# nibox/Pose-Estimation-with-Message-Passing-Networks

Measured on AMD Instinct MI355X. Metric: images/sec (640px, HRNet-w48) + MPN edge-updates/sec at 1/2/4/8 MI355X, higher is better.
Workload: dtype f16x3; 1 GPU; c3: 8x17x640x640 heatmaps/GPU -> fully graph -> MPN TypeAware-attn T=3; images_per_gpu=8, global_batch=8, persons_per_image=9, nodes_per_gpu=1224, edges_per_gpu=186048, parallelism=image-sharded x1, batches_in_flight=2, detection_and_node_math=fp32

## Files before the change

### pose-estimation-with-message-passing-networks_amd/csrc/mpn.hip

```cpp
#include <limits.h>

#include <algorithm>
#include <atomic>
#include <type_traits>
#include <map>
#include <mutex>
#include <string>
#include <vector>
#include <string.h>
#include <math.h>

#include "pemp_common.h"

namespace pemp {
namespace {

constexpr int D = 64;
constexpr int LDW = 72;
constexpr int MAXT = 17;
constexpr int EDGE_WAVES = 16;
constexpr int EMB_WAVES = 16, EMB_PER_CU = 1;
constexpr int EMB_MIN_WAVES_EU = EMB_WAVES * EMB_PER_CU / 4 > 1 ? EMB_WAVES * EMB_PER_CU / 4 : 1;
constexpr int RESERVE_CUS_DEFAULT = 64;
constexpr int64_t RESERVE_MIN_EDGES = 65536;
// ... 477 lines not shown
      : "=&v"(hi), "=&v"(lo)
      : "v"(x0), "v"(x1), "v"(s));
}

__device__ __forceinline__ float frag_absmax(const float (&x)[4][4]) {
  float m = 0.0f;
#pragma unroll
  for (int b = 0; b < 4; ++b) m = fmaxf(m, fmaxf(fmaxf(fabsf(x[b][0]), fabsf(x[b][1])), fmaxf(fabsf(x[b][2]), fabsf(x[b][3]))));
  return m;
}

__device__ __forceinline__ bool f16_big(const float (&x)[4][4], float s) {
  return __any(!(frag_absmax(x) * s < F16_BIG));
}

__device__ __forceinline__ float f16_item_scale(float m, float s) {
  m = xmax_rows(m);
  m *= s;
  if (m < F16_BIG) return 1.0f;
  if (!(m <= 3.4028235e38f)) return F16_DOWN;
  int e;
  frexpf(m, &e);
  return ldexpf(1.0f, 14 - e);
}

__device__ __forceinline__ float frag_max_nonneg(const float (&x)[4][4]) {
  int m = 0;
#pragma unroll
  for (int b = 0; b < 4; ++b)
    m = max(m, max(max(__float_as_int(x[b][0]), __float_as_int(x[b][1])), max(__float_as_int(x[b][2]), __float_as_int(x[b][3]))));
  return __int_as_float(m);
}

template <bool NONNEG = false>
__device__ __forceinline__ bool split_f16(const float (&x)[4][4], float s, f16x8_t (&hi)[2], f16x8_t (&lo)[2],
                                          float& sc, float extra = 1.0f) {
  const float m = NONNEG ? frag_max_nonneg(x) : frag_absmax(x);
  const bool big = __any(!(m * s < F16_BIG));
  sc = big ? f16_item_scale(m, s) : 1.0f;
  const float ss = s * sc * extra;
#pragma unroll
  for (int kb = 0; kb < 2; ++kb) {
    uint32_t h[4], l[4];
#pragma unroll
    for (int d = 0; d < 4; ++d)
      split_pair(x[2 * kb + (d >> 1)][2 * (d & 1)], x[2 * kb + (d >> 1)][2 * (d & 1) + 1], ss, h[d], l[d]);
    const u32x4_t hv = {h[0], h[1], h[2], h[3]}, lv = {l[0], l[1], l[2], l[3]};
    hi[kb] = __builtin_bit_cast(f16x8_t, hv);
    lo[kb] = __builtin_bit_cast(f16x8_t, lv);
  }
  return big;
}

template <int OB, bool BIG>
__device__ __forceinline__ void gemm_h3_body(const _Float16* W, const f16x8_t (&hi)[2],
                                             const f16x8_t (&lo)[2], float sc, float (&acc)[OB][4]) {
  const int lane = __lane_id(), i = lane & 15, g = lane >> 4;
  const float isc = BIG ? 1.0f / sc : 1.0f;
#pragma unroll
  for (int ob = 0; ob < OB; ++ob) {
    f32x4 c = {acc[ob][0], acc[ob][1], acc[ob][2], acc[ob][3]};
    if (BIG) c *= sc;
#pragma unroll
    for (int kb = 0; kb < 2; ++kb) {
      const int o = (16 * ob + i) * 2 * LDW + 32 * kb + 8 * g;
      const f16x8_t ah = *reinterpret_cast<const f16x8_t*>(W + o);
      const f16x8_t al = *reinterpret_cast<const f16x8_t*>(W + o + 64);
      c = __builtin_amdgcn_mfma_f32_16x16x32_f16(al, hi[kb], c, 0, 0, 0);
      c = __builtin_amdgcn_mfma_f32_16x16x32_f16(ah, lo[kb], c, 0, 0, 0);
      c = __builtin_amdgcn_mfma_f32_16x16x32_f16(ah, hi[kb], c, 0, 0, 0);
    }
    if (BIG) c *= isc;
    acc[ob][0] = c[0]; acc[ob][1] = c[1]; acc[ob][2] = c[2]; acc[ob][3] = c[3];
  }
}

template <int OB>
__device__ __forceinline__ void gemm_h3(const _Float16* W, const f16x8_t (&hi)[2], const f16x8_t (&lo)[2],
                                        bool big, float sc, float (&acc)[OB][4]) {
  if (__builtin_expect(big, 0)) gemm_h3_body<OB, true>(W, hi, lo, sc, acc);
  else gemm_h3_body<OB, false>(W, hi, lo, 1.0f, acc);
}

template <int PREC>
struct Frag {
  bf16x8_t bh[2], bl[2];
  f16x8_t hh[2], hl[2];
  bool big;
  float sc;
};

template <int PREC, bool NONNEG = false>
__device__ __forceinline__ void prep(const float (&x)[4][4], Frag<PREC>& f) {
  if constexpr (PREC == 1) split_bf16(x, f.bh, f.bl);
  else if constexpr (PREC == 2) f.big = split_f16<NONNEG>(x, dom_inv<PREC>(), f.hh, f.hl, f.sc);
}

template <bool NONNEG = false>
__device__ __forceinline__ void prep_f16_scaled(const float (&x)[4][4], Frag<2>& f, float extra) {
  f.big = split_f16<NONNEG>(x, dom_inv<2>(), f.hh, f.hl, f.sc, extra);
}

template <int PREC>
__device__ __forceinline__ void prep_true(const float (&x)[4][4], Frag<PREC>& f) {
  if constexpr (PREC == 1) split_bf16(x, f.bh, f.bl);
  else if constexpr (PREC == 2) f.big = split_f16(x, 1.0f, f.hh, f.hl, f.sc);
}

template <int PREC, int OB>
__device__ __forceinline__ void gemm_f(const void* W, const float (&x)[4][4], const Frag<PREC>& f, float (&acc)[OB][4]) {
  if constexpr (PREC == 0) gemm_frag<4, OB>(static_cast<const float*>(W), LDW, x, acc);
  else if constexpr (PREC == 1) gemm_bf3<OB>(static_cast<const __bf16*>(W), f.bh, f.bl, acc);
  else gemm_h3<OB>(static_cast<const _Float16*>(W), f.hh, f.hl, f.big, f.sc, acc);
}

__device__ __forceinline__ int interleaved_slot(int row, int rows_per_part, int ld, int part_len) {
  const int part = row >= rows_per_part, r = row - part * rows_per_part;
  return r * ld + part * part_len;
}

__host__ __device__ constexpr int lds_stride(int in_pad) { return (in_pad - 8 + 63) / 64 * 64 + 8; }

struct EmbedLayout {
  int n, prec, w_off[5], stride[5], kb[5], ob[5], b_off[5], relu[5], g_off[5], total;
};

__host__ __device__ constexpr int lds_stride_bf(int in_pad) { return 2 * in_pad + 16; }

__host__ __device__ constexpr EmbedLayout embed_layout_dims(int n, const int* in_dim, const int* out_dim, const int* relu,
                                                            int prec) {
  EmbedLayout L{};
  L.n = n;
  L.prec = prec;
  int off = 0, goff = 0;
  for (int l = 0; l <= L.n; ++l) {
    const int in = l < L.n ? in_dim[l] : 64, out = l < L.n ? out_dim[l] : 64;
    L.ob[l] = (out + 15) / 16;
    L.relu[l] = l < L.n ? relu[l] : 0;
    L.w_off[l] = off;
    if (prec != PEMP_PREC_FP32) {
      L.kb[l] = (in + 31) / 32;
      L.stride[l] = lds_stride_bf(32 * L.kb[l]);
      off += 16 * L.ob[l] * L.stride[l] / 2;
      L.g_off[l] = goff;
      goff += 2 * 16 * L.ob[l] * 32 * L.kb[l];
    } else {
      L.kb[l] = (in + 15) / 16;
      L.stride[l] = lds_stride(16 * L.kb[l]);
      off += 16 * L.ob[l] * L.stride[l];
    }
  }
  for (int l = 0; l <= L.n; ++l) {
    L.b_off[l] = off;
    off += 16 * L.ob[l];
  }
  L.total = off;
  return L;
}

static EmbedLayout embed_layout(const pemp_mlp& m, int prec) {
  int in[4] = {}, out[4] = {}, relu[4] = {};
  const int n = m.n_layers < 4 ? m.n_layers : 4;
  for (int l = 0; l < n; ++l) {
    in[l] = m.layer[l].in_dim;
    out[l] = m.layer[l].out_dim;
    relu[l] = m.layer[l].relu;
// ... 205 lines not shown
          c = __builtin_amdgcn_mfma_f32_16x16x32_bf16(ah, hb[kb], c, 0, 0, 0);
        } else {
          const f16x8_t ah = *reinterpret_cast<const f16x8_t*>(W + o);
          const f16x8_t al = *reinterpret_cast<const f16x8_t*>(W + o + lo_off);
          c = __builtin_amdgcn_mfma_f32_16x16x32_f16(al, hh[kb], c, 0, 0, 0);
          c = __builtin_amdgcn_mfma_f32_16x16x32_f16(ah, lh[kb], c, 0, 0, 0);
          c = __builtin_amdgcn_mfma_f32_16x16x32_f16(ah, hh[kb], c, 0, 0, 0);
        }
      }
#pragma unroll
      for (int r = 0; r < 4; ++r) {
        const float v = c[r] * s_out;
        out[ob][r] = relu ? fmaxf(v, 0.0f) : v;
      }
    } else {
#pragma unroll
      for (int r = 0; r < 4; ++r) out[ob][r] = 0.0f;
    }
  }
}

template <int KB, bool NONNEG>
__device__ __forceinline__ bool split_f16_kb(const float (&x)[4][4], float s, f16x8_t (&hi)[2], f16x8_t (&lo)[2],
                                             float& sc) {
  float m;
  if constexpr (NONNEG) {
    int mi = 0;
#pragma unroll
    for (int b = 0; b < 2 * KB; ++b)
      mi = max(mi, max(max(__float_as_int(x[b][0]), __float_as_int(x[b][1])), max(__float_as_int(x[b][2]), __float_as_int(x[b][3]))));
    m = __int_as_float(mi);
  } else {
    m = 0.0f;
#pragma unroll
    for (int b = 0; b < 2 * KB; ++b)
      m = fmaxf(m, fmaxf(fmaxf(fabsf(x[b][0]), fabsf(x[b][1])), fmaxf(fabsf(x[b][2]), fabsf(x[b][3]))));
  }
  const bool big = __any(!(m * s < F16_BIG));
  sc = big ? f16_item_scale(m, s) : 1.0f;
  const float ss = s * sc;
#pragma unroll
  for (int kb = 0; kb < KB; ++kb) {
    uint32_t h[4], l[4];
#pragma unroll
    for (int d = 0; d < 4; ++d)
      split_pair(x[2 * kb + (d >> 1)][2 * (d & 1)], x[2 * kb + (d >> 1)][2 * (d & 1) + 1], ss, h[d], l[d]);
    const u32x4_t hv = {h[0], h[1], h[2], h[3]}, lv = {l[0], l[1], l[2], l[3]};
    hi[kb] = __builtin_bit_cast(f16x8_t, hv);
    lo[kb] = __builtin_bit_cast(f16x8_t, lv);
  }
  return big;
}

template <int KB32, int OB, bool RELU, bool NONNEG, bool BIG>
__device__ __forceinline__ void layer_h3_body(const _Float16* W, int ldw, const float* bias, const f16x8_t (&hh)[2],
                                              const f16x8_t (&lh)[2], float sc, float (&out)[4][4]) {
  const int lane = __lane_id(), i = lane & 15, g = lane >> 4;
  constexpr int lo_off = 32 * KB32;
  const float isc = BIG ? 1.0f / sc : 1.0f;
#pragma unroll
  for (int ob = 0; ob < 4; ++ob) {
    if (ob < OB) {
      const float4 bb = ld4(bias + 16 * ob + 4 * g);
      f32x4 c = {bb.x, bb.y, bb.z, bb.w};
      if (BIG) c *= sc;
#pragma unroll
      for (int kb = 0; kb < KB32; ++kb) {
        const int o = (16 * ob + i) * ldw + 32 * kb + 8 * g;
        const f16x8_t ah = *reinterpret_cast<const f16x8_t*>(W + o);
        const f16x8_t al = *reinterpret_cast<const f16x8_t*>(W + o + lo_off);
        c = __builtin_amdgcn_mfma_f32_16x16x32_f16(al, hh[kb], c, 0, 0, 0);
        c = __builtin_amdgcn_mfma_f32_16x16x32_f16(ah, lh[kb], c, 0, 0, 0);
        c = __builtin_amdgcn_mfma_f32_16x16x32_f16(ah, hh[kb], c, 0, 0, 0);
      }
      if (BIG) c *= isc;
#pragma unroll
      for (int r = 0; r < 4; ++r) out[ob][r] = RELU ? fmaxf(c[r], 0.0f) : c[r];
    } else {
#pragma unroll
      for (int r = 0; r < 4; ++r) out[ob][r] = 0.0f;
    }
  }
}

template <int KB32, int OB, bool RELU, bool NONNEG, bool IN_DOM>
__device__ __forceinline__ void layer_h3(const float* smz, const EmbedLayout& Lo, int l, const float (&in)[4][4],
                                         float (&out)[4][4], Frag<2>* split_out = nullptr) {
  const _Float16* W = reinterpret_cast<const _Float16*>(smz + Lo.w_off[l]);
  const float* bias = smz + Lo.b_off[l];
  f16x8_t hh[2], lh[2];
  float sc;
  const bool big = split_f16_kb<KB32, NONNEG>(in, IN_DOM ? dom_inv<2>() : 1.0f, hh, lh, sc);
  if (split_out) {
    split_out->hh[0] = hh[0]; split_out->hh[1] = hh[1];
    split_out->hl[0] = lh[0]; split_out->hl[1] = lh[1];
    split_out->big = big;
    split_out->sc = sc;
  }
  if (__builtin_expect(big, 0)) layer_h3_body<KB32, OB, RELU, NONNEG, true>(W, Lo.stride[l], bias, hh, lh, sc, out);
  else layer_h3_body<KB32, OB, RELU, NONNEG, false>(W, Lo.stride[l], bias, hh, lh, 1.0f, out);
}

template <int PREC, bool COMP = false>
__device__ __forceinline__ void embed_tile_fixed(const float* smz, const EmbedLayout& Lo, float (&x)[4][4],
                                                 float (&y)[4][4], Frag<PREC>& fx) {
  if constexpr (PREC == 2 && COMP) {
    layer_h3<1, 2, true, false, false>(smz, Lo, 0, x, y);
    layer_h3<1, 4, true, true, true>(smz, Lo, 1, y, x);
    layer_h3<2, 4, true, true, true>(smz, Lo, 2, x, y);
    layer_h3<2, 4, false, true, true>(smz, Lo, 3, y, x, &fx);
  } else if constexpr (PREC == 2) {
    layer_h3<1, 2, true, false, false>(smz, Lo, 0, x, y);
    layer_h3<1, 4, true, true, true>(smz, Lo, 1, y, x);
    layer_h3<2, 4, true, true, true>(smz, Lo, 2, x, y);
    layer_h3<2, 4, false, true, true>(smz, Lo, 3, y, x);
    layer_h3<2, 4, false, false, true>(smz, Lo, 4, x, y, &fx);
  } else {
    layer_fixed<PREC, 1, 2>(smz, Lo, 0, x, y);
    layer_fixed<PREC, 1, 4>(smz, Lo, 1, y, x);
    layer_fixed<PREC, 2, 4>(smz, Lo, 2, x, y);
    layer_fixed<PREC, 2, 4>(smz, Lo, 3, y, x);
    layer_fixed<PREC, 2, 4, true>(smz, Lo, 4, x, y, &fx);
  }
}

static bool embed_fixed_shape(const EmbedLayout& L) {
  static const int kb[5] = {1, 1, 2, 2, 2}, ob[5] = {2, 4, 4, 4, 4}, relu[5] = {1, 1, 1, 0, 0};
  if (L.prec == PEMP_PREC_FP32 || L.n != 4) return false;
  for (int l = 0; l < 5; ++l)
    if (L.kb[l] != kb[l] || L.ob[l] != ob[l] || (L.relu[l] != 0) != (relu[l] != 0)) return false;
  return true;
}
static bool embed_composed(const EmbedLayout& L, int prec, const pemp_mpn_weights& w) {
  return prec == PEMP_PREC_F16X3 && embed_fixed_shape(L) && w.emb_comp_bf && w.emb_comp_b;
}

template <int PREC>
__device__ __forceinline__ void stage_tile64(float* dst, const float* w32, int64_t ld32, const uint16_t* wbf) {
  if (PREC == 0) {
    for (int idx = threadIdx.x; idx < D * 16; idx += blockDim.x) {
      const int row = idx >> 4, c4 = (idx & 15) * 4;
      *reinterpret_cast<float4*>(&dst[row * LDW + c4]) = ld4(w32 + row * ld32 + c4);
    }
  } else {
    __bf16* db = reinterpret_cast<__bf16*>(dst);
    for (int idx = threadIdx.x; idx < 2 * D * 8; idx += blockDim.x) {
      const int row = idx >> 3, c8 = (idx & 7) * 8;
      *reinterpret_cast<uint4*>(&db[interleaved_slot(row, D, 2 * LDW, D) + c8]) =
          *reinterpret_cast<const uint4*>(wbf + row * D + c8);
    }
  }
}

template <int PREC, bool FIXED>
__device__ __forceinline__ void embed_stage(float* dst, int tid, int nthreads, const pemp_mlp& emb, const EmbedLayout& Lo,
                                            const uint16_t* __restrict__ emb_bf, const float* __restrict__ q0_w,
                                            const float* __restrict__ q0_b, const float* __restrict__ e1_w,
                                            const uint16_t* __restrict__ e1_bf, const uint16_t* __restrict__ comp_bf,
                                            const float* __restrict__ comp_b) {
  const bool comp = FIXED && PREC == 2 && comp_bf && comp_b;
  float* d64 = dst + Lo.total;
  if (comp) {
  } else if (PREC == 0) {
    for (int idx = tid; idx < D * 16; idx += nthreads) {
      const int row = idx >> 4, c4 = (idx & 15) * 4;
      *reinterpret_cast<float4*>(&d64[row * LDW + c4]) = ld4(e1_w + row * D + c4);
    }
  } else {
    __bf16* db = reinterpret_cast<__bf16*>(d64);
// ... 49 lines not shown
void edge_embed_kernel(pemp_mlp emb, EmbedLayout Lo,
                                                                     const uint16_t* __restrict__ emb_bf,
                                                                     const float* __restrict__ ea, int A,
                                                                     const int* __restrict__ s_orig, int64_t E,
                                                                     const float* __restrict__ q0_w,
                                                                     const float* __restrict__ q0_b,
                                                                     const float* __restrict__ e1_w,
                                                                     const uint16_t* __restrict__ e1_bf,
                                                                     float* __restrict__ r0, float* __restrict__ q0,
                                                                     const int64_t* __restrict__ ne,
                                                                     const float* __restrict__ img,
                                                                     const uint16_t* __restrict__ comp_bf,
                                                                     const float* __restrict__ comp_b) {
  constexpr bool FIXED = FX >= 1, COMP = FX == 2;
  extern __shared__ __attribute__((aligned(16))) float sm[];
  if (ne) E = ne[1];
  const int lane = threadIdx.x & 63, wave = threadIdx.x >> 6, c = lane & 15, g = lane >> 4;
  if (img) {
    dma_to_lds(sm, img, COMP ? embed_comp_floats(Lo) : embed_image_floats(Lo));
    lds_drain();
  } else {
    embed_stage<PREC, FIXED>(sm, threadIdx.x, 64 * EMB_WAVES, emb, Lo, emb_bf, q0_w, q0_b, e1_w, e1_bf,
                             COMP ? comp_bf : nullptr, COMP ? comp_b : nullptr);
  }
  __syncthreads();
  const int64_t gw = (int64_t)blockIdx.x * EMB_WAVES + wave, nw = (int64_t)gridDim.x * EMB_WAVES;
  const int first = __builtin_amdgcn_readfirstlane((int)(E * gw / nw));
  const int end = __builtin_amdgcn_readfirstlane((int)(E * (gw + 1) / nw));
  const rsrc_t rs_ea = make_rsrc(ea, (int)E * A * 4), rs_orig = make_rsrc(s_orig, (int)E * 4);
  const rsrc_t rs_q0 = make_rsrc(q0, (int)E * 256), rs_r0 = make_rsrc(r0, (int)E * 256);
  int o_next = first < end ? bld1(rs_orig, 4 * min(first + c, end - 1)) : 0;
  float ea_n[2][4];
  if (FIXED && first < end) {
    load_edge_attr32(rs_ea, A, o_next, ea_n);
    o_next = bld1(rs_orig, 4 * min(first + 16 + c, end - 1));
  }
  for (int base = first; base < end; base += 16) {
    int z = 0;
    asm volatile("" : "+s"(z));
    const float* smz = sm + z;
    const int p = base + c;
    const bool valid = p < end;
    float x[4][4], y[4][4];
    if constexpr (FIXED) {
      ea_mask(A, ea_n, x);
      load_edge_attr32(rs_ea, A, o_next, ea_n);
      o_next = bld1(rs_orig, 4 * min(base + 32 + c, end - 1));
    } else {
      const int o = o_next;
      o_next = bld1(rs_orig, 4 * min(base + 16 + c, end - 1));
      load_edge_attr(rs_ea, A, o, x);
    }
    Frag<PREC> fx;
    const int vo = valid ? p * 256 + 16 * g : OOB_VOFF;
    if constexpr (COMP) {
      embed_tile_fixed<PREC, true>(smz, Lo, x, y, fx);
#pragma unroll
      for (int ob = 0; ob < 4; ++ob) bst4(rs_q0, vo + 64 * ob, x[ob][0], x[ob][1], x[ob][2], x[ob][3]);
      const float* br = smz + Lo.b_off[4];
#pragma unroll
      for (int ob = 0; ob < 4; ++ob) {
        const float4 bb = ld4(br + 16 * ob + 4 * g);
        x[ob][0] = bb.x; x[ob][1] = bb.y; x[ob][2] = bb.z; x[ob][3] = bb.w;
      }
      gemm_f<PREC, 4>(smz + Lo.w_off[4], y, fx, x);
#pragma unroll
      for (int ob = 0; ob < 4; ++ob) bst4(rs_r0, vo + 64 * ob, x[ob][0], x[ob][1], x[ob][2], x[ob][3]);
      continue;
    }
    if constexpr (FIXED) {
      embed_tile_fixed<PREC>(smz, Lo, x, y, fx);
    } else {
      embed_tile<PREC>(smz, Lo, x, y);
      if (PREC == 2) {
#pragma unroll
        for (int ob = 0; ob < 4; ++ob)
#pragma unroll
          for (int r = 0; r < 4; ++r) y[ob][r] *= dom<PREC>();
      }
      prep_true<PREC>(x, fx);
    }
#pragma unroll
    for (int ob = 0; ob < 4; ++ob) bst4(rs_q0, vo + 64 * ob, y[ob][0], y[ob][1], y[ob][2], y[ob][3]);
    gemm_f<PREC, 4>(smz + Lo.total, x, fx, y);
#pragma unroll
    for (int ob = 0; ob < 4; ++ob) bst4(rs_r0, vo + 64 * ob, y[ob][0], y[ob][1], y[ob][2], y[ob][3]);
  }
}

struct EdgeStepArgs {
  int64_t N, E;
  int T, t_nt_ld;
  const int4* ranges;
  const int *s_src, *s_dst, *s_orig;
  const float *NT, *Q0, *r_cur;
  float* r_next;
  const float* img;
  int64_t img_stride;
  float* agg;
  pemp_mlp head;
  float* edge_logits;
  int write_next;
  unsigned long long* stamps;
  const int64_t* ne;
  int rec;
  const float* ea;
  int A;
  const float* emb_img;
};

#ifdef PEMP_STAMPS
#define EDGE_STAMP(k)                                                                               \
  do {                                                                                              \
    if (a.stamps && lane == 0) {                                                                    \
      unsigned long long t_;                                                                        \
      asm volatile("s_memrealtime %0\n\ts_waitcnt lgkmcnt(0)" : "=s"(t_)::"memory");                \
      a.stamps[16 * ((int64_t)blockIdx.x * NW + wave) + (k)] = t_;                                  \
    }                                                                                               \
  } while (0)
#else
#define EDGE_STAMP(k) \
  do {                \
  } while (0)
#endif
// ... 377 lines not shown
  if (FIRST && first < end) o_next = bld1(rs_orig, 4 * min(first + c, end - 1));
  {
    const float* src = a.img + (int64_t)t * a.img_stride + SKIP;
    constexpr int PIECES = IMG_F / 256, TAIL = IMG_F - PIECES * 256;
    for (int k = wave; k < PIECES; k += NW)
      dma16(src + 256 * k + 4 * lane, img + 256 * k);
    if (TAIL && wave == NW - 1 && 4 * lane < TAIL)
      *reinterpret_cast<float4*>(&img[256 * PIECES + 4 * lane]) = ld4(src + 256 * PIECES + 4 * lane);
    if constexpr (FIRST) {
      constexpr int EP = EMB_F / 256, ET = EMB_F - EP * 256;
      for (int k = wave; k < EP; k += NW) dma16(a.emb_img + 256 * k + 4 * lane, rbuf + 256 * k);
      if (ET && wave == NW - 2 && 4 * lane < ET)
        *reinterpret_cast<float4*>(&rbuf[256 * EP + 4 * lane]) = ld4(a.emb_img + 256 * EP + 4 * lane);
    }
  }
  if (FIRST) {
    if (first < end) {
      load_edge_attr32(rs_ea, a.A, o_next, ea_n);
      o_next = bld1(rs_orig, 4 * min(first + 16 + c, end - 1));
    }
  } else if (first < end) {
    gather_nt(dst_n, src_n, true);
    dma_rows(rs_r, first, mybuf, lane);
    if (HEAD == 1) orig_t = bld1(rs_orig, 4 * min(first + c, end - 1));
  }
  __syncthreads();
  EDGE_STAMP(1);
  EDGE_STAMP(2);
  const int seg_first = (rflags & RANGE_CONT_IN) ? sdst_id(__builtin_amdgcn_readfirstlane(dst_n)) : -1;
  const rsrc_t rs_next = make_rsrc(a.r_next, E * 256);
  const rsrc_t rs_agg = make_rsrc(a.agg, (int)a.N * T * 256);
  const u32x4v_s rw_r = rsrc_words(a.r_cur, end * 256);
  const u32x4v_s rw_q = rsrc_words(a.Q0, end * 256);
  const rsrc_t rs_q0 = make_rsrc(a.Q0, FIRST ? E * 256 : 0);
  const bool store_next = MID && a.write_next;

  float cacc[4][4];
  float cM = 0.f, cl = 0.f;
  bool have_carry = false;
  int tile_no = 0;
  for (int base = first; base < end; base += 16, ++tile_no) {
    if (tile_no < 4) EDGE_STAMP(3 + 3 * tile_no);
    if (tile_no == 0) __builtin_amdgcn_s_setprio(3);
    else if (tile_no == 1) __builtin_amdgcn_s_setprio(2);
    else if (tile_no == 2) __builtin_amdgcn_s_setprio(1);
    else if (tile_no == 3) __builtin_amdgcn_s_setprio(0);
    int z = 0;
    asm volatile("" : "+s"(z));
    const float* W1 = img + z;
    const float* W2 = img + z + D * LDW - SKIP;
    const float* WM = img + z + 2 * D * LDW - SKIP;
    const float* UW = img + z + 3 * D * LDW - SKIP;
    const float* hwz = hw + z;
    const int p = base + c;
    const bool valid = p < end;
    const int dst = dst_n, src = src_n;
    const bool more = base + 16 < end;
    dst_n = dst_nn;
    src_n = src_nn;
    constexpr int NG = 12 + (HEAD == 1 ? 1 : 0);
    if (!FIRST && tile_no > 0) {
      if (store_next) dma_wait<8 + NG>();
      else dma_wait<4 + NG>();
    }
    float h[4][4], m[4][4], q0r[4][4];
    float4 rr[4];
    if constexpr (FIRST) {
      const float* smz = rbuf + z;
      float y[4][4], r0[4][4];
      Frag<PREC> fx;
      ea_mask(a.A, ea_n, q0r, g + z);
      load_edge_attr32(rs_ea, a.A, o_next, ea_n, g + z);
      o_next = bld1(rs_orig, 4 * min(base + 32 + c, end - 1));
      embed_tile_fixed<PREC, true>(smz, ELO, q0r, y, fx);
      const int vq0 = valid ? p * 256 + 16 * g : OOB_VOFF;
#pragma unroll
      for (int ob = 0; ob < 4; ++ob) bst4(rs_q0, vq0 + 64 * ob, q0r[ob][0], q0r[ob][1], q0r[ob][2], q0r[ob][3]);
      gather_ab(dst, src);
      const float* br = smz + ELO.b_off[4];
#pragma unroll
      for (int ob = 0; ob < 4; ++ob) {
        const float4 bb = ld4(br + 16 * ob + 4 * g);
        r0[ob][0] = bb.x; r0[ob][1] = bb.y; r0[ob][2] = bb.z; r0[ob][3] = bb.w;
      }
      gemm_f<PREC, 4>(smz + ELO.w_off[4], y, fx, r0);
#pragma unroll
      for (int ob = 0; ob < 4; ++ob) rr[ob] = make_float4(r0[ob][0], r0[ob][1], r0[ob][2], r0[ob][3]);
    } else {
      const int cz = c + z, rowb = 64 * cz + 4 * g;
#pragma unroll
      for (int ob = 0; ob < 4; ++ob) rr[ob] = ld4(mybuf + (rowb ^ (16 * (ob ^ (cz & 3)))));
    }
    const int vq = p * 256 + 16 * g;
    const int orig = orig_t;
    if (MID && !FIRST) {
#pragma unroll
      for (int ob = 0; ob < 4; ++ob) asm volatile("" ::"v"(xa[ob].x), "v"(xb[ob].x), "v"(xp[ob].x));
      if (store_next) dma_rows_async(rw_q, base, mybuf, lane);
    }
    {
      const int qn = min(base + 32 + c, end - 1);
      dst_nn = bld1(rs_dst, 4 * qn);
      src_nn = bld1(rs_src, 4 * qn);
    }
    float ab[4][4];
#pragma unroll
    for (int ob = 0; ob < 4; ++ob) {
      if (EPT) {
        h[ob][0] = rr[ob].x; h[ob][1] = rr[ob].y; h[ob][2] = rr[ob].z; h[ob][3] = rr[ob].w;
        ab[ob][0] = xa[ob].x + xb[ob].x; ab[ob][1] = xa[ob].y + xb[ob].y;
        ab[ob][2] = xa[ob].z + xb[ob].z; ab[ob][3] = xa[ob].w + xb[ob].w;
      } else {
        h[ob][0] = rr[ob].x + xa[ob].x + xb[ob].x; h[ob][1] = rr[ob].y + xa[ob].y + xb[ob].y;
        h[ob][2] = rr[ob].z + xa[ob].z + xb[ob].z; h[ob][3] = rr[ob].w + xa[ob].w + xb[ob].w;
      }
    }
    if constexpr (FIRST) {
#pragma unroll
      for (int ob = 0; ob < 4; ++ob) asm volatile("" ::"v"(h[ob][0]), "v"(h[ob][1]), "v"(h[ob][2]), "v"(h[ob][3]));
      gather_p(dst);
#pragma unroll
      for (int ob = 0; ob < 4; ++ob) {
        const float4 q = bld4(rs_q0, min(p, end - 1) * 256 + 16 * g + 64 * ob);
        q0r[ob][0] = q.x; q0r[ob][1] = q.y; q0r[ob][2] = q.z; q0r[ob][3] = q.w;
      }
    }
    if (!MID) {
#pragma unroll
      for (int ob = 0; ob < 4; ++ob) asm volatile("" ::"v"(xa[ob].x), "v"(xb[ob].x), "v"(xp[ob].x));
      if (HEAD == 1) asm volatile("" ::"v"(orig));
      if (more) dma_rows_async(rw_r, base + 16, mybuf, lane);
    }
#pragma unroll
    for (int ob = 0; ob < 4; ++ob) {
      m[ob][0] = xp[ob].x; m[ob][1] = xp[ob].y; m[ob][2] = xp[ob].z; m[ob][3] = xp[ob].w;
    }
#ifdef PEMP_STAMPS
    asm volatile("" ::"v"(h[0][0]), "v"(h[3][3]));
    if (tile_no < 4) EDGE_STAMP(4 + 3 * tile_no);
#endif
    relu_frag<4>(h);
    float ep[4][4];
#pragma unroll
    for (int ob = 0; ob < 4; ++ob) {
      const float4 b2 = ld4(vec + 16 * ob + 4 * g);
      ep[ob][0] = b2.x; ep[ob][1] = b2.y; ep[ob][2] = b2.z; ep[ob][3] = b2.w;
      if (EPT) { ep[ob][0] += ab[ob][0]; ep[ob][1] += ab[ob][1]; ep[ob][2] += ab[ob][2]; ep[ob][3] += ab[ob][3]; }
    }
    {
      Frag<PREC> fh;
      prep<PREC, true>(h, fh);
      gemm_f<PREC, 4>(W2, h, fh, ep);
    }
    relu_frag<4>(ep);
    float av = 0.f;
    if (AGG == PEMP_AGGR_ATTN) {
#pragma unroll
      for (int ob = 0; ob < 4; ++ob) {
        const float4 w = ld4(vec + D + 16 * ob + 4 * g);
        av = fmaf(w.x, ep[ob][0], av); av = fmaf(w.y, ep[ob][1], av);
        av = fmaf(w.z, ep[ob][2], av); av = fmaf(w.w, ep[ob][3], av);
      }
      av = xsum_rows(av);
      av += vec[z + 2 * D];
    }
    const int seg = valid ? sdst_id(dst) : -1 - c;
    const Chunks ck = chunks_of(dst, c, min(end - 1 - base, 15), valid);
    const bool carry_in = have_carry;
    float M = 0.f, pe = 1.0f;
    if (AGG == PEMP_AGGR_ATTN) {
#if PEMP_ASM_SCANS
      M = chunk_max_asm(av, chunk_masks(ck));
#else
      M = seg_bcast_tail_max(seg_max(av, ck.d), ck.u);
#endif
      if (carry_in && ck.d == c) M = fmaxf(M, cM);
      pe = pemp_exp(av - M);
    }
    if (HEAD == 2) {
      float h1[4][4], h2[4][4];
#pragma unroll
      for (int ob = 0; ob < 4; ++ob)
#pragma unroll
        for (int r = 0; r < 4; ++r) h1[ob][r] = ep[ob][r] * dom_inv<PREC>();
      mlp_frag<4>(a.head, h1, h2);
      if (valid && g == 0)
        __builtin_amdgcn_raw_buffer_store_b32(__float_as_uint(h1[0][0]), make_rsrc(logits, E * 4),
                                              4 * a.s_orig[p], 0, 0);
    }
    Frag<PREC> fe;
    prep<PREC, true>(ep, fe);
    if (MID && !FIRST) {
      if (store_next) {
        dma_wait<2>();
        const int cz = c + z, rowb = 64 * cz + 4 * g;
#pragma unroll
        for (int ob = 0; ob < 4; ++ob) {
          const float4 q = ld4(mybuf + (rowb ^ (16 * (ob ^ (cz & 3)))));
          q0r[ob][0] = q.x; q0r[ob][1] = q.y; q0r[ob][2] = q.z; q0r[ob][3] = q.w;
        }
      }
      if (more) dma_rows_async(rw_r, base + 16, mybuf, lane);
    }
    if (MID && a.write_next) {
      gemm_f<PREC, 4>(W1, ep, fe, q0r);
      const int vn = valid ? vq : OOB_VOFF;
#pragma unroll
      for (int ob = 0; ob < 4; ++ob) bst4(rs_next, vn + 64 * ob, q0r[ob][0], q0r[ob][1], q0r[ob][2], q0r[ob][3]);
    }
    if (HEAD == 1) {
      const float* hb = hb_l + z;
      float h1[4][4], h2[2][4];
#pragma unroll
      for (int ob = 0; ob < 4; ++ob) {
        const float4 bb = ld4(hb + 16 * ob + 4 * g);
        h1[ob][0] = bb.x; h1[ob][1] = bb.y; h1[ob][2] = bb.z; h1[ob][3] = bb.w;
      }
      gemm_f<PREC, 4>(hwz, ep, fe, h1);
      relu_frag<4>(h1);
#pragma unroll
      for (int ob = 0; ob < 2; ++ob) {
        const float4 bb = ld4(hb + D + 16 * ob + 4 * g);
        h2[ob][0] = bb.x; h2[ob][1] = bb.y; h2[ob][2] = bb.z; h2[ob][3] = bb.w;
      }
      {
        Frag<PREC> f1;
        prep<PREC, true>(h1, f1);
        gemm_f<PREC, 2>(hwz + D * LDW, h1, f1, h2);
      }
      relu_frag<2>(h2);
      float lg = 0.f;
#pragma unroll
      for (int ob = 0; ob < 2; ++ob) {
        const float4 w = ld4(hb + D + 32 + 16 * ob + 4 * g);
        lg = fmaf(w.x, h2[ob][0], lg); lg = fmaf(w.y, h2[ob][1], lg);
        lg = fmaf(w.z, h2[ob][2], lg); lg = fmaf(w.w, h2[ob][3], lg);
      }
      lg = xsum_rows(lg);
      if (valid && g == 0)
        __builtin_amdgcn_raw_buffer_store_b32(__float_as_uint(lg + hb[D + 64]), make_rsrc(logits, E * 4),
                                              4 * orig, 0, 0);
    }
    gemm_f<PREC, 4>(WM, ep, fe, m);
    relu_frag<4>(m);
    if (UPD) {
      float u[4][4];
#pragma unroll
      for (int ob = 0; ob < 4; ++ob)
#pragma unroll
        for (int r = 0; r < 4; ++r) u[ob][r] = 0.0f;
      Frag<PREC> fm;
      if constexpr (PE_FOLD) prep_f16_scaled<true>(m, fm, pe);
      else prep<PREC, true>(m, fm);
      gemm_f<PREC, 4>(UW, m, fm, u);
#pragma unroll
      for (int ob = 0; ob < 4; ++ob)
#pragma unroll
        for (int r = 0; r < 4; ++r) m[ob][r] = u[ob][r];
    }

    float l = (AGG == PEMP_AGGR_ATTN) ? pe : 1.0f;
    float v[4][4];
#pragma unroll
    for (int ob = 0; ob < 4; ++ob)
#pragma unroll
      for (int r = 0; r < 4; ++r) v[ob][r] = (AGG == PEMP_AGGR_ATTN && !PE_FOLD) ? pe * m[ob][r] : m[ob][r];
    if (carry_in && c == 0) {
      if (AGG == PEMP_AGGR_ATTN) {
        const float f = pemp_exp(cM - M);
        l += cl * f;
#pragma unroll
        for (int ob = 0; ob < 4; ++ob)
#pragma unroll
          for (int r = 0; r < 4; ++r) v[ob][r] = fmaf(cacc[ob][r], f, v[ob][r]);
      } else {
        l += cl;
#pragma unroll
        for (int ob = 0; ob < 4; ++ob)
#pragma unroll
          for (int r = 0; r < 4; ++r)
            v[ob][r] = (AGG == PEMP_AGGR_MAX) ? fmaxf(v[ob][r], cacc[ob][r]) : v[ob][r] + cacc[ob][r];
      }
    }
    const ScanMask smk = scan_mask(ck.d);
    {
      if (AGG == PEMP_AGGR_ATTN || AGG == PEMP_AGGR_MEAN) l = seg_sum(l, smk);
#pragma unroll
      for (int ob = 0; ob < 4; ++ob)
#pragma unroll
        for (int r = 0; r < 4; ++r) v[ob][r] = (AGG == PEMP_AGGR_MAX) ? seg_max(v[ob][r], ck.d) : seg_sum(v[ob][r], smk);
    }
    const int seg15 = __builtin_amdgcn_readlane(seg, 15);
    const bool carry_out = more && sdst_id(__builtin_amdgcn_readlane(dst_n, 0)) == seg15;
    if (carry_out) {
      cl = readlane_f(l, 15);
      cM = readlane_f(M, 15);
#pragma unroll
      for (int ob = 0; ob < 4; ++ob)
#pragma unroll
        for (int r = 0; r < 4; ++r) cacc[ob][r] = dppf<DPP_SHL15>(v[ob][r], 0.0f);
    }
    have_carry = carry_out;
    {
      const float inv = ((AGG == PEMP_AGGR_ATTN) ? pemp_rcp(l + 1e-12f) : (AGG == PEMP_AGGR_MEAN) ? pemp_rcp(l) : 1.0f) *
                        dom_inv<PREC>();
      const bool out = valid && ck.tail && !(carry_out && c == 15);
      const bool pin = seg == seg_first;
// ... 2393 lines not shown
```

Baseline: 35510 images/s.

## Software-pipeline LDS weight fragment reads across chained f16x3 MFMA GEMMs

Restructures the f16x3 split-precision GEMM so that weight fragments for the next step are read from LDS while the current MFMAs run. The first fragment of the following layer's weights is also prefetched across GEMM boundaries in both the embedding MLP and the edge update chain. sched_group_barrier hints interleave ds_reads with MFMAs. The big-scale path becomes a runtime multiply instead of a separate template instantiation. This aims to hide LDS latency between dependent MFMA chains, at the cost of higher VGPR pressure from holding prefetched fragments, which could lower occupancy.

```diff
diff --git a/pose-estimation-with-message-passing-networks_amd/csrc/mpn.hip b/pose-estimation-with-message-passing-networks_amd/csrc/mpn.hip
--- a/pose-estimation-with-message-passing-networks_amd/csrc/mpn.hip
+++ b/pose-estimation-with-message-passing-networks_amd/csrc/mpn.hip
@@ -553,34 +553,68 @@
   return big;
 }
 
-template <int OB, bool BIG>
-__device__ __forceinline__ void gemm_h3_body(const _Float16* W, const f16x8_t (&hi)[2],
-                                             const f16x8_t (&lo)[2], float sc, float (&acc)[OB][4]) {
+struct H3Step {
+  f16x8_t ah[2], al[2];
+};
+__device__ __forceinline__ void h3_read(const _Float16* W, int ldw, int lo_off, int q, int kb, H3Step& f) {
   const int lane = __lane_id(), i = lane & 15, g = lane >> 4;
-  const float isc = BIG ? 1.0f / sc : 1.0f;
+  const int o = (32 * q + i) * ldw + 32 * kb + 8 * g;
+#pragma unroll
+  for (int j = 0; j < 2; ++j) f.al[j] = *reinterpret_cast<const f16x8_t*>(W + o + 16 * j * ldw + lo_off);
+#pragma unroll
+  for (int j = 0; j < 2; ++j) f.ah[j] = *reinterpret_cast<const f16x8_t*>(W + o + 16 * j * ldw);
+}
+
+template <int KB, int OB, bool PRE, bool NEXT>
+__device__ __forceinline__ void h3_chain(const _Float16* W, int ldw, int lo_off, const f16x8_t (&hi)[2],
+                                         const f16x8_t (&lo)[2], f32x4 (&c)[OB], H3Step& io,
+                                         const _Float16* Wn, int ldwn, int lo_offn) {
+  static_assert(OB % 2 == 0, "two output blocks per step");
+  constexpr int Q = OB / 2, S = KB * Q;
+  H3Step f[S + 1];
+  if (PRE) f[0] = io;
+  else h3_read(W, ldw, lo_off, 0, 0, f[0]);
+#pragma unroll
+  for (int s = 0; s < S; ++s) {
+    const int kb = s / Q, q = s % Q;
+    if (s + 1 < S) h3_read(W, ldw, lo_off, (s + 1) % Q, (s + 1) / Q, f[s + 1]);
+    else if (NEXT) h3_read(Wn, ldwn, lo_offn, 0, 0, f[s + 1]);
+#pragma unroll
+    for (int j = 0; j < 2; ++j) c[2 * q + j] = __builtin_amdgcn_mfma_f32_16x16x32_f16(f[s].al[j], hi[kb], c[2 * q + j], 0, 0, 0);
+#pragma unroll
+    for (int j = 0; j < 2; ++j) c[2 * q + j] = __builtin_amdgcn_mfma_f32_16x16x32_f16(f[s].ah[j], lo[kb], c[2 * q + j], 0, 0, 0);
+#pragma unroll
+    for (int j = 0; j < 2; ++j) c[2 * q + j] = __builtin_amdgcn_mfma_f32_16x16x32_f16(f[s].ah[j], hi[kb], c[2 * q + j], 0, 0, 0);
+    constexpr int MFMA = 0x008, DS_READ = 0x100;
+    const bool rd = s + 1 < S || NEXT;
+    __builtin_amdgcn_sched_group_barrier(MFMA, 2, 0);
+    if (rd) __builtin_amdgcn_sched_group_barrier(DS_READ, 2, 0);
+    __builtin_amdgcn_sched_group_barrier(MFMA, 4, 0);
+    if (rd) __builtin_amdgcn_sched_group_barrier(DS_READ, 2, 0);
+  }
+  if (NEXT) io = f[S];
+}
+
+template <int OB, bool PRE = false, bool NEXT = false>
+__device__ __forceinline__ void gemm_h3(const _Float16* W, const f16x8_t (&hi)[2], const f16x8_t (&lo)[2],
+                                        bool big, float sc, float (&acc)[OB][4], H3Step& io, const _Float16* Wn) {
+  f32x4 c[OB];
+#pragma unroll
+  for (int ob = 0; ob < OB; ++ob) c[ob] = f32x4{acc[ob][0], acc[ob][1], acc[ob][2], acc[ob][3]};
+  if (__builtin_expect(big, 0)) {
+#pragma unroll
+    for (int ob = 0; ob < OB; ++ob) c[ob] *= sc;
+  }
+  h3_chain<2, OB, PRE, NEXT>(W, 2 * LDW, 64, hi, lo, c, io, Wn, 2 * LDW, 64);
+  if (__builtin_expect(big, 0)) {
+    const float isc = 1.0f / sc;
+#pragma unroll
+    for (int ob = 0; ob < OB; ++ob) c[ob] *= isc;
+  }
 #pragma unroll
   for (int ob = 0; ob < OB; ++ob) {
-    f32x4 c = {acc[ob][0], acc[ob][1], acc[ob][2], acc[ob][3]};
-    if (BIG) c *= sc;
-#pragma unroll
-    for (int kb = 0; kb < 2; ++kb) {
-      const int o = (16 * ob + i) * 2 * LDW + 32 * kb + 8 * g;
-      const f16x8_t ah = *reinterpret_cast<const f16x8_t*>(W + o);
-      const f16x8_t al = *reinterpret_cast<const f16x8_t*>(W + o + 64);
-      c = __builtin_amdgcn_mfma_f32_16x16x32_f16(al, hi[kb], c, 0, 0, 0);
-      c = __builtin_amdgcn_mfma_f32_16x16x32_f16(ah, lo[kb], c, 0, 0, 0);
-      c = __builtin_amdgcn_mfma_f32_16x16x32_f16(ah, hi[kb], c, 0, 0, 0);
-    }
-    if (BIG) c *= isc;
-    acc[ob][0] = c[0]; acc[ob][1] = c[1]; acc[ob][2] = c[2]; acc[ob][3] = c[3];
-  }
-}
-
-template <int OB>
-__device__ __forceinline__ void gemm_h3(const _Float16* W, const f16x8_t (&hi)[2], const f16x8_t (&lo)[2],
-                                        bool big, float sc, float (&acc)[OB][4]) {
-  if (__builtin_expect(big, 0)) gemm_h3_body<OB, true>(W, hi, lo, sc, acc);
-  else gemm_h3_body<OB, false>(W, hi, lo, 1.0f, acc);
+    acc[ob][0] = c[ob][0]; acc[ob][1] = c[ob][1]; acc[ob][2] = c[ob][2]; acc[ob][3] = c[ob][3];
+  }
 }
 
 template <int PREC>
@@ -612,7 +646,28 @@
 __device__ __forceinline__ void gemm_f(const void* W, const float (&x)[4][4], const Frag<PREC>& f, float (&acc)[OB][4]) {
   if constexpr (PREC == 0) gemm_frag<4, OB>(static_cast<const float*>(W), LDW, x, acc);
   else if constexpr (PREC == 1) gemm_bf3<OB>(static_cast<const __bf16*>(W), f.bh, f.bl, acc);
-  else gemm_h3<OB>(static_cast<const _Float16*>(W), f.hh, f.hl, f.big, f.sc, acc);
+  else {
+    H3Step io;
+    gemm_h3<OB>(static_cast<const _Float16*>(W), f.hh, f.hl, f.big, f.sc, acc, io, nullptr);
+  }
+}
+
+template <int PREC, bool AHEAD = true>
+struct WPre {
+  H3Step s;
+};
+template <int PREC, bool AHEAD>
+__device__ __forceinline__ void wpre(const void* W, WPre<PREC, AHEAD>& p) {
+  if constexpr (PREC == 2 && AHEAD) h3_read(static_cast<const _Float16*>(W), 2 * LDW, 64, 0, 0, p.s);
+}
+
+template <int PREC, int OB, bool NEXT, bool AHEAD>
+__device__ __forceinline__ void gemm_fp(const void* W, const float (&x)[4][4], const Frag<PREC>& f, float (&acc)[OB][4],
+                                        WPre<PREC, AHEAD>& p, const void* Wn = nullptr) {
+  if constexpr (PREC == 2 && AHEAD)
+    gemm_h3<OB, true, NEXT>(static_cast<const _Float16*>(W), f.hh, f.hl, f.big, f.sc, acc, p.s,
+                            static_cast<const _Float16*>(Wn));
+  else gemm_f<PREC, OB>(W, x, f, acc);
 }
 
 __device__ __forceinline__ int interleaved_slot(int row, int rows_per_part, int ld, int part_len) {
@@ -924,40 +979,39 @@
   return big;
 }
 
-template <int KB32, int OB, bool RELU, bool NONNEG, bool BIG>
+template <int KB32, int OB, bool RELU, int KBN>
 __device__ __forceinline__ void layer_h3_body(const _Float16* W, int ldw, const float* bias, const f16x8_t (&hh)[2],
-                                              const f16x8_t (&lh)[2], float sc, float (&out)[4][4]) {
-  const int lane = __lane_id(), i = lane & 15, g = lane >> 4;
-  constexpr int lo_off = 32 * KB32;
-  const float isc = BIG ? 1.0f / sc : 1.0f;
-#pragma unroll
-  for (int ob = 0; ob < 4; ++ob) {
-    if (ob < OB) {
-      const float4 bb = ld4(bias + 16 * ob + 4 * g);
-      f32x4 c = {bb.x, bb.y, bb.z, bb.w};
-      if (BIG) c *= sc;
-#pragma unroll
-      for (int kb = 0; kb < KB32; ++kb) {
-        const int o = (16 * ob + i) * ldw + 32 * kb + 8 * g;
-        const f16x8_t ah = *reinterpret_cast<const f16x8_t*>(W + o);
-        const f16x8_t al = *reinterpret_cast<const f16x8_t*>(W + o + lo_off);
-        c = __builtin_amdgcn_mfma_f32_16x16x32_f16(al, hh[kb], c, 0, 0, 0);
-        c = __builtin_amdgcn_mfma_f32_16x16x32_f16(ah, lh[kb], c, 0, 0, 0);
-        c = __builtin_amdgcn_mfma_f32_16x16x32_f16(ah, hh[kb], c, 0, 0, 0);
-      }
-      if (BIG) c *= isc;
-#pragma unroll
-      for (int r = 0; r < 4; ++r) out[ob][r] = RELU ? fmaxf(c[r], 0.0f) : c[r];
-    } else {
-#pragma unroll
-      for (int r = 0; r < 4; ++r) out[ob][r] = 0.0f;
-    }
-  }
-}
-
-template <int KB32, int OB, bool RELU, bool NONNEG, bool IN_DOM>
+                                              const f16x8_t (&lh)[2], bool big, float sc, float (&out)[4][4],
+                                              H3Step& io, const _Float16* Wn, int ldwn) {
+  const int lane = __lane_id(), g = lane >> 4;
+  f32x4 c[OB];
+#pragma unroll
+  for (int ob = 0; ob < OB; ++ob) {
+    const float4 bb = ld4(bias + 16 * ob + 4 * g);
+    c[ob] = f32x4{bb.x, bb.y, bb.z, bb.w};
+  }
+  if (__builtin_expect(big, 0)) {
+#pragma unroll
+    for (int ob = 0; ob < OB; ++ob) c[ob] *= sc;
+  }
+  h3_chain<KB32, OB, true, (KBN > 0)>(W, ldw, 32 * KB32, hh, lh, c, io, Wn, ldwn, 32 * KBN);
+  if (__builtin_expect(big, 0)) {
+    const float isc = 1.0f / sc;
+#pragma unroll
+    for (int ob = 0; ob < OB; ++ob) c[ob] *= isc;
+  }
+#pragma unroll
+  for (int ob = 0; ob < 4; ++ob)
+#pragma unroll
+    for (int r = 0; r < 4; ++r) {
+      const float v = c[ob < OB ? ob : 0][r];
+      out[ob][r] = ob < OB ? (RELU ? fmaxf(v, 0.0f) : v) : 0.0f;
+    }
+}
+
+template <int KB32, int OB, bool RELU, bool NONNEG, bool IN_DOM, int KBN>
 __device__ __forceinline__ void layer_h3(const float* smz, const EmbedLayout& Lo, int l, const float (&in)[4][4],
-                                         float (&out)[4][4], Frag<2>* split_out = nullptr) {
+                                         float (&out)[4][4], H3Step& io, Frag<2>* split_out = nullptr) {
   const _Float16* W = reinterpret_cast<const _Float16*>(smz + Lo.w_off[l]);
   const float* bias = smz + Lo.b_off[l];
   f16x8_t hh[2], lh[2];
@@ -969,24 +1023,28 @@
     split_out->big = big;
     split_out->sc = sc;
   }
-  if (__builtin_expect(big, 0)) layer_h3_body<KB32, OB, RELU, NONNEG, true>(W, Lo.stride[l], bias, hh, lh, sc, out);
-  else layer_h3_body<KB32, OB, RELU, NONNEG, false>(W, Lo.stride[l], bias, hh, lh, 1.0f, out);
+  const int ln = KBN > 0 ? l + 1 : l;
+  layer_h3_body<KB32, OB, RELU, KBN>(W, Lo.stride[l], bias, hh, lh, big, sc, out, io,
+                                     reinterpret_cast<const _Float16*>(smz + Lo.w_off[ln]), Lo.stride[ln]);
 }
 
 template <int PREC, bool COMP = false>
 __device__ __forceinline__ void embed_tile_fixed(const float* smz, const EmbedLayout& Lo, float (&x)[4][4],
-                                                 float (&y)[4][4], Frag<PREC>& fx) {
+                                                 float (&y)[4][4], Frag<PREC>& fx, WPre<PREC>& wp) {
+  if constexpr (PREC == 2) {
+    h3_read(reinterpret_cast<const _Float16*>(smz + Lo.w_off[0]), Lo.stride[0], 32, 0, 0, wp.s);
+  }
   if constexpr (PREC == 2 && COMP) {
-    layer_h3<1, 2, true, false, false>(smz, Lo, 0, x, y);
-    layer_h3<1, 4, true, true, true>(smz, Lo, 1, y, x);
-    layer_h3<2, 4, true, true, true>(smz, Lo, 2, x, y);
-    layer_h3<2, 4, false, true, true>(smz, Lo, 3, y, x, &fx);
+    layer_h3<1, 2, true, false, false, 1>(smz, Lo, 0, x, y, wp.s);
+    layer_h3<1, 4, true, true, true, 2>(smz, Lo, 1, y, x, wp.s);
+    layer_h3<2, 4, true, true, true, 2>(smz, Lo, 2, x, y, wp.s);
+    layer_h3<2, 4, false, true, true, 2>(smz, Lo, 3, y, x, wp.s, &fx);
   } else if constexpr (PREC == 2) {
-    layer_h3<1, 2, true, false, false>(smz, Lo, 0, x, y);
-    layer_h3<1, 4, true, true, true>(smz, Lo, 1, y, x);
-    layer_h3<2, 4, true, true, true>(smz, Lo, 2, x, y);
-    layer_h3<2, 4, false, true, true>(smz, Lo, 3, y, x);
-    layer_h3<2, 4, false, false, true>(smz, Lo, 4, x, y, &fx);
+    layer_h3<1, 2, true, false, false, 1>(smz, Lo, 0, x, y, wp.s);
+    layer_h3<1, 4, true, true, true, 2>(smz, Lo, 1, y, x, wp.s);
+    layer_h3<2, 4, true, true, true, 2>(smz, Lo, 2, x, y, wp.s);
+    layer_h3<2, 4, false, true, true, 2>(smz, Lo, 3, y, x, wp.s);
+    layer_h3<2, 4, false, false, true, 0>(smz, Lo, 4, x, y, wp.s, &fx);
   } else {
     layer_fixed<PREC, 1, 2>(smz, Lo, 0, x, y);
     layer_fixed<PREC, 1, 4>(smz, Lo, 1, y, x);
@@ -1142,9 +1200,10 @@
       load_edge_attr(rs_ea, A, o, x);
     }
     Frag<PREC> fx;
+    WPre<PREC> wp;
     const int vo = valid ? p * 256 + 16 * g : OOB_VOFF;
     if constexpr (COMP) {
-      embed_tile_fixed<PREC, true>(smz, Lo, x, y, fx);
+      embed_tile_fixed<PREC, true>(smz, Lo, x, y, fx, wp);
 #pragma unroll
       for (int ob = 0; ob < 4; ++ob) bst4(rs_q0, vo + 64 * ob, x[ob][0], x[ob][1], x[ob][2], x[ob][3]);
       const float* br = smz + Lo.b_off[4];
@@ -1153,13 +1212,13 @@
         const float4 bb = ld4(br + 16 * ob + 4 * g);
         x[ob][0] = bb.x; x[ob][1] = bb.y; x[ob][2] = bb.z; x[ob][3] = bb.w;
       }
-      gemm_f<PREC, 4>(smz + Lo.w_off[4], y, fx, x);
+      gemm_fp<PREC, 4, false>(smz + Lo.w_off[4], y, fx, x, wp);
 #pragma unroll
       for (int ob = 0; ob < 4; ++ob) bst4(rs_r0, vo + 64 * ob, x[ob][0], x[ob][1], x[ob][2], x[ob][3]);
       continue;
     }
     if constexpr (FIXED) {
-      embed_tile_fixed<PREC>(smz, Lo, x, y, fx);
+      embed_tile_fixed<PREC>(smz, Lo, x, y, fx, wp);
     } else {
       embed_tile<PREC>(smz, Lo, x, y);
       if (PREC == 2) {
@@ -1643,6 +1702,7 @@
     const float* WM = img + z + 2 * D * LDW - SKIP;
     const float* UW = img + z + 3 * D * LDW - SKIP;
     const float* hwz = hw + z;
+    const float* WA = HEAD == 1 ? hwz : WM;
     const int p = base + c;
     const bool valid = p < end;
     const int dst = dst_n, src = src_n;
@@ -1656,6 +1716,7 @@
     }
     float h[4][4], m[4][4], q0r[4][4];
     float4 rr[4];
+    WPre<PREC, !EPT && HEAD != 2> wp;
     if constexpr (FIRST) {
       const float* smz = rbuf + z;
       float y[4][4], r0[4][4];
@@ -1663,7 +1724,7 @@
       ea_mask(a.A, ea_n, q0r, g + z);
       load_edge_attr32(rs_ea, a.A, o_next, ea_n, g + z);
       o_next = bld1(rs_orig, 4 * min(base + 32 + c, end - 1));
-      embed_tile_fixed<PREC, true>(smz, ELO, q0r, y, fx);
+      embed_tile_fixed<PREC, true>(smz, ELO, q0r, y, fx, wp);
       const int vq0 = valid ? p * 256 + 16 * g : OOB_VOFF;
 #pragma unroll
       for (int ob = 0; ob < 4; ++ob) bst4(rs_q0, vq0 + 64 * ob, q0r[ob][0], q0r[ob][1], q0r[ob][2], q0r[ob][3]);
@@ -1674,7 +1735,7 @@
         const float4 bb = ld4(br + 16 * ob + 4 * g);
         r0[ob][0] = bb.x; r0[ob][1] = bb.y; r0[ob][2] = bb.z; r0[ob][3] = bb.w;
       }
-      gemm_f<PREC, 4>(smz + ELO.w_off[4], y, fx, r0);
+      gemm_fp<PREC, 4, true>(smz + ELO.w_off[4], y, fx, r0, wp, W2);
 #pragma unroll
       for (int ob = 0; ob < 4; ++ob) rr[ob] = make_float4(r0[ob][0], r0[ob][1], r0[ob][2], r0[ob][3]);
     } else {
@@ -1730,6 +1791,7 @@
     asm volatile("" ::"v"(h[0][0]), "v"(h[3][3]));
     if (tile_no < 4) EDGE_STAMP(4 + 3 * tile_no);
 #endif
+    if (!FIRST) wpre(W2, wp);
     relu_frag<4>(h);
     float ep[4][4];
 #pragma unroll
@@ -1741,7 +1803,7 @@
     {
       Frag<PREC> fh;
       prep<PREC, true>(h, fh);
-      gemm_f<PREC, 4>(W2, h, fh, ep);
+      gemm_fp<PREC, 4, true>(W2, h, fh, ep, wp, MID ? W1 : WA);
     }
     relu_frag<4>(ep);
     float av = 0.f;
@@ -1793,11 +1855,15 @@
       }
       if (more) dma_rows_async(rw_r, base + 16, mybuf, lane);
     }
+    constexpr bool W1_NEXT = FIRST || HEAD == 1;
     if (MID && a.write_next) {
-      gemm_f<PREC, 4>(W1, ep, fe, q0r);
+      gemm_fp<PREC, 4, W1_NEXT>(W1, ep, fe, q0r, wp, WA);
       const int vn = valid ? vq : OOB_VOFF;
 #pragma unroll
       for (int ob = 0; ob < 4; ++ob) bst4(rs_next, vn + 64 * ob, q0r[ob][0], q0r[ob][1], q0r[ob][2], q0r[ob][3]);
+      if (!W1_NEXT) wpre(WA, wp);
+    } else if (MID) {
+      wpre(WA, wp);
     }
     if (HEAD == 1) {
       const float* hb = hb_l + z;
@@ -1807,7 +1873,7 @@
         const float4 bb = ld4(hb + 16 * ob + 4 * g);
         h1[ob][0] = bb.x; h1[ob][1] = bb.y; h1[ob][2] = bb.z; h1[ob][3] = bb.w;
       }
-      gemm_f<PREC, 4>(hwz, ep, fe, h1);
+      gemm_fp<PREC, 4, true>(hwz, ep, fe, h1, wp, hwz + D * LDW);
       relu_frag<4>(h1);
 #pragma unroll
       for (int ob = 0; ob < 2; ++ob) {
@@ -1817,7 +1883,7 @@
       {
         Frag<PREC> f1;
         prep<PREC, true>(h1, f1);
-        gemm_f<PREC, 2>(hwz + D * LDW, h1, f1, h2);
+        gemm_fp<PREC, 2, true>(hwz + D * LDW, h1, f1, h2, wp, WM);
       }
       relu_frag<2>(h2);
       float lg = 0.f;
@@ -1832,7 +1898,7 @@
         __builtin_amdgcn_raw_buffer_store_b32(__float_as_uint(lg + hb[D + 64]), make_rsrc(logits, E * 4),
                                               4 * orig, 0, 0);
     }
-    gemm_f<PREC, 4>(WM, ep, fe, m);
+    gemm_fp<PREC, 4, (UPD != 0)>(WM, ep, fe, m, wp, UW);
     relu_frag<4>(m);
     if (UPD) {
       float u[4][4];
@@ -1843,7 +1909,7 @@
       Frag<PREC> fm;
       if constexpr (PE_FOLD) prep_f16_scaled<true>(m, fm, pe);
       else prep<PREC, true>(m, fm);
-      gemm_f<PREC, 4>(UW, m, fm, u);
+      gemm_fp<PREC, 4, false>(UW, m, fm, u, wp);
 #pragma unroll
       for (int ob = 0; ob < 4; ++ob)
 #pragma unroll
```

Result: no change. 35650 images/s, median of 2 (+0.4%).
